# flare-rpc/flare-cpp

Hardware: AMD Instinct MI355X
Metric: GiB/s device-resident Snappy decode+encode, batched RPC bodies, 1/2/4/8 GPU (higher is better)
Workload: dtype u8; 1 GPU; C3 decompress: 65,536 x 64 KiB Zipf-text bodies (~2.0x), device-resident; op=decompress, messages_rank0=65536, global_batch=65536, raw_bytes_all_ranks=4294967296, compressed_bytes_all_ranks=2134156024, parallelism=shard1 (weak: messages by index; no data-path collective), world_size_seen_by_collectives=1

## Files before the change

### flare-cpp_amd/csrc/decode_v4_exec5.h

```cpp
#pragma once

#include "decode_v4_exec_common.h"
#include "decode_v4_plan.h"
#include "snappy_pieces.h"
#include "wave_util.h"

namespace fsg {

namespace {
constexpr u32 kGroupBytes = 1024;

__device__ __forceinline__ u32 exec_tag_entry(u32 c) {
  const u32 type = c & 3, l0 = (c >> 2) + 1;
  u32 nb, len, lit = 0, ll = 0, hi = 0;
  if (type == 0) {
    lit = 1;
    nb = l0 > 60 ? l0 - 60 : 0;
    ll = nb ? 1 : 0;
    len = nb ? 0 : l0;
  } else if (type == 1) {
    nb = 1;
    len = 4 + ((c >> 2) & 7);
    hi = (c >> 5) << 8;
  } else {
    nb = type == 2 ? 2 : 4;
    len = l0;
  }
  return ((32 - 8 * nb) & 31) | (ll << 5) | (lit << 6) | (len << 8) | (nb << 16) | (hi << 20);
}
}

__device__ __forceinline__ void exec5_message(
    u32 m, const u8* __restrict__ in, const u64* __restrict__ in_off,
    const u32* __restrict__ in_len, u8* out, const u64* __restrict__ out_off,
    const u32* __restrict__ out_len, i32* __restrict__ status, const u32* __restrict__ bm_base,
    const u32* __restrict__ bitmap, u32* ring, const u32* tagtab, u8* sb, const u32x4* sel_tab,
    const u32x4* mtab, u32 lane, i32 st, u32 ip0, u32 op0, u32 op1, bool prio, u32 keep_hist) {
  const u32 bmb = bm_base[m];
  const u32 n_in = in_len[m];
  const u32 expected = out_len[m];
  const u8* ib = in + in_off[m];
  u8* ob = out + out_off[m];
  if (st != kOk) return;
  const u32 ibal = (u32)(reinterpret_cast<uintptr_t>(ib) & 15);
  const u32 obal = (u32)(reinterpret_cast<uintptr_t>(ob) & 15);
  const __amdgpu_buffer_rsrc_t irsrc = msg_rsrc(ib - ibal, ibal + n_in);
  const __amdgpu_buffer_rsrc_t orsrc =
      __builtin_amdgcn_make_buffer_rsrc(ob - obal, (short)0, (int)(expected + obal), 0x00020000);

  if ((bmb & kSingleLiteral) && op1 == expected && op0 == 0) {
    const u32 S = bmb & ~kSingleLiteral;
    for (u32 k0 = 0; k0 < expected; k0 += 4096) {
      Raw16 x[4];
#pragma unroll
      for (u32 r = 0; r < 4; ++r) x[r] = raw_load16(irsrc, S + k0 + 1024 * r + lane * 16 + ibal);
#pragma unroll
      for (u32 r = 0; r < 4; ++r) {
        const u32 k = k0 + 1024 * r + lane * 16;
        if (k < expected) store_exact(ob + k, shifted16(x[r]), expected - k < 16 ? expected - k : 16u);
      }
    }
    return;
  }
  const u32* bm = bitmap + bmb;
  const u32 nwords = (n_in + 31) >> 5;
#ifdef FSG_STAMPS
  u64 st_[8] = {0, 0, 0, 0, 0, 0, 0, 0};
  u64 t_last_ = __builtin_amdgcn_s_memtime();
#endif

  u32 head = 0, tail = 0, scan = ip0 >> 5, op = op0;
  int sbase = (int)((op0 + obal) & ~15u) - (int)obal;
  u32 flushed = op0;
  auto zero_from = [&](u32 from) {
    const u32 i = from + 16 * lane;
    if (i < kWindow + 32) *reinterpret_cast<u32x4*>(sb + i) = u32x4{0, 0, 0, 0};
  };
  zero_from(0);
  u32 zero_end = 1024;
  wave_lds_fence();
  auto fill_word = [&](u32 sc) -> u32 {
    const u32 wi = sc + (lane >> 2);
    return (lane < 4 * kFillWords && wi < nwords) ? bm[wi] : 0u;
  };
  u32 bmw = fill_word(scan);
  u32 pf_head = 0xffffffffu, pf_cnt = 0;
  u32 pf_pos = 0;
  u32x4 pd = u32x4{0, 0, 0, 0};
  u32 pd4 = 0;
  auto prefetch = [&](u32 p) {
    const u32 a = (p + ibal) & ~3u;
    pd = __builtin_amdgcn_raw_buffer_load_b128(irsrc, a, 0, 0);
    pd4 = __builtin_amdgcn_raw_buffer_load_b32(irsrc, a + 16, 0, 0);
  };

  auto flush_to = [&](u32 fe) {
    if (fe <= flushed) return;
    const int b0 = (int)(((flushed + obal) & ~15u)) - (int)obal;
    for (int blk = b0 + 16 * (int)lane; blk < (int)fe; blk += 1024) {
      const u32 lo = blk < (int)flushed ? flushed : (u32)blk;
      const u32 hi = blk + 16 < (int)fe ? (u32)(blk + 16) : fe;
      if (hi - lo == 16) {
        const u32x4 v = *reinterpret_cast<const u32x4*>(sb + (blk - sbase));
        __builtin_memcpy(ob + blk, &v, 16);
      } else {
        store_exact(ob + lo, lds_read16(sb + ((int)lo - sbase)), hi - lo);
      }
    }
    flushed = fe;
  };

  for (;;) {
    if (tail - head < 2 * kMaxPieces && scan < nwords) {
      if (prio) __builtin_amdgcn_s_setprio(1);
      u32 bits = (bmw >> (8 * (lane & 3))) & 0xffu;
      const u32 bitbase = (scan + (lane >> 2)) * 32 + 8 * (lane & 3);
      if (bitbase < ip0) bits &= bitbase + 8 <= ip0 ? 0u : (0xffu << (ip0 - bitbase)) & 0xffu;
      const u32 cnt = __builtin_popcount(bits);
      const u32 incl = dpp_incl_scan(cnt);
      u32 slot = tail + incl - cnt;
      while (bits) {
        ring[slot & (kTagRing - 1)] = bitbase + __builtin_ctz(bits);
        ++slot;
        bits &= bits - 1;
      }
      tail += readlane(incl, 63);
      scan += kFillWords;
      bmw = fill_word(scan);
      wave_lds_fence();
      STAMP(0);
      continue;
    }
    const u32 avail = tail - head;
    if (avail == 0 || op >= op1) break;
    const u32 take0 = avail < 64 ? avail : 64u;
    const bool valid = lane < take0;
    const u32 pos = ring[(head + lane) & (kTagRing - 1)];
    if (pf_head != head || pf_cnt < take0) prefetch(pos);
    if (prio) __builtin_amdgcn_s_setprio(1);

    const u32 s = (pos + ibal) & 3u;
    const u32 c = __builtin_amdgcn_alignbyte(pd[1], pd[0], s) & 0xffu;
    const u32 e = tagtab[c];
    const bool q = s == 3;
    const u32 w0 = q ? pd[1] : pd[0], w1 = q ? pd[2] : pd[1], w2 = q ? pd[3] : pd[2];
    const u32 w3 = q ? pd4 : pd[3];
    const u32 b = (s + 1) & 3u;
    const u32x4 xr = u32x4{__builtin_amdgcn_alignbyte(w1, w0, b), __builtin_amdgcn_alignbyte(w2, w1, b),
                           __builtin_amdgcn_alignbyte(w3, w2, b), __builtin_amdgcn_alignbyte(pd4, w3, b)};
    const u32 val = xr[0] & (0xffffffffu >> (e & 31u));
    const bool is_lit = e & 64u;
    const u32 len = (e & 32u) ? val + 1u : (e >> 8) & 0x7fu;
    const u32 off = val + (e >> 20);
    const u32 nb = (e >> 16) & 7u;
    const u32 lsrc = pos + 1 + nb;

    const u64 bigm = __ballot(valid && is_lit && len > 64);
    STAMP(1);
    if (bigm & 1ull) {
      const u32 L = readlane(len, 0), S = readlane(lsrc, 0);
      if ((u64)op + L > op1) {
        if (lane == 0) status[m] = kCorrupt;
        return;
      }
      flush_to(op);
      for (u32 k0 = 0; k0 < L; k0 += 4096) {
        Raw16 x[4];
#pragma unroll
        for (u32 r = 0; r < 4; ++r) x[r] = raw_load16(irsrc, S + k0 + 1024 * r + lane * 16 + ibal);
#pragma unroll
        for (u32 r = 0; r < 4; ++r) {
          const u32 k = k0 + 1024 * r + lane * 16;
          if (k < L) store_exact(ob + op + k, shifted16(x[r]), L - k < 16 ? L - k : 16u);
        }
      }
      op += L;
      flushed = op;
      sbase = (int)((op + obal) & ~15u) - (int)obal - 16;
      zero_from(0);
      zero_end = 1024;
      wave_lds_fence();
      if (lane < 2) {
        const u32 lo = (u32)sbase + 16 * lane;
        if (lo < op) {
          const u32 cnt = op - lo < 16 ? op - lo : 16u;
          store_exact(sb + 16 * lane, rsrc_load16(irsrc, S + L - (op - lo) + ibal), cnt);
        }
      }
      wave_lds_fence();
      head += 1;
      pf_head = 0xffffffffu;
      if (head == tail) {
        const u32 nw = (S + L) >> 5;
        if (nw > scan) {
          scan = nw;
          bmw = fill_word(scan);
        }
      }
      STAMP(7);
      continue;
    }
    const u32 take = bigm ? (u32)__builtin_ctzll(bigm) : take0;
    const bool v = lane < take;

    const u32 lv = v ? len : 0u;
    const u32 incl = dpp_incl_scan(lv);
    const u32 t_op = op + incl - lv;
    const bool fits = v && incl <= kGroupBytes && t_op < op1;
    const u32 k_tags = (u32)__builtin_popcountll(__ballot(fits));
    const u32 tot_len = readlane(incl, k_tags - 1);
    if (__any(fits && (len > op1 - t_op || (!is_lit && (off == 0 || off > t_op - op0))))) {
      if (lane == 0) status[m] = kCorrupt;
      return;
    }

    if (op + tot_len - sbase > kWindow) {
      const int nsb = (int)(((op - keep_hist + obal) & ~15u)) - (int)obal;
      if ((int)flushed < nsb + 16) flush_to((u32)((int)((op + obal) & ~15u) - (int)obal));
      wait_all_memory();
      const u32 shift = (u32)(nsb - sbase), keep = (u32)((int)op - nsb);
      for (u32 k = 0; k < keep; k += 1024) {
        const u32 i = k + 16 * lane;
        u32x4 x = u32x4{0, 0, 0, 0};
        if (i < keep) x = *reinterpret_cast<const u32x4*>(sb + shift + i);
        wave_lds_fence();
        if (i < keep) *reinterpret_cast<u32x4*>(sb + i) = x;
        wave_lds_fence();
      }
      sbase = nsb;
      zero_end = (keep + 15) & ~15u;
    }
    auto prefetch_next_and_zero = [&]() {
      {
        const u32 nh = head + k_tags;
        const u32 na = tail - nh;
        const u32 ncnt = na < 64 ? na : 64u;
        pf_pos = ring[(nh + lane) & (kTagRing - 1)];
        prefetch(pf_pos);
        pf_head = nh;
        pf_cnt = ncnt;
      }
      while (op + tot_len + 20 - sbase > zero_end) {
        zero_from(zero_end);
        zero_end += 1024;
      }
      wave_lds_fence();
    };

    STAMP(2);
    const u32 src = is_lit ? lsrc : t_op - off;
    const u32 nch = (len + 15) >> 4;
    const bool pat = !is_lit && off < 16 && off < len;
    const u32 below = (u32)(sbase - (int)src);
    const u32 kfar = (int)below > 0 ? ((below - 1) >> 4) + 1 : 0u;
    const u32 kready = src + len <= op ? nch : (src < op ? (op - src) >> 4 : 0u);
    const u32 klead = kfar > kready ? kfar : kready;
    const u32 kc = pat ? 0u : (klead < nch ? klead : nch);
    const u32 kf = fits ? (is_lit ? nch : kc) : 0u;
    const bool reg0 = is_lit && nb == 0;
    const u32 sh = is_lit ? (src + ibal) & 3u : 0u;
    auto gload = [&](u32 k, u32x4& d, u32& d4) {
      if (is_lit) {
        const u32 a = (src + 16 * k + ibal) & ~3u;
        d = __builtin_amdgcn_raw_buffer_load_b128(irsrc, a, 0, 0);
        d4 = __builtin_amdgcn_raw_buffer_load_b32(irsrc, a + 16, 0, 0);
      } else if (k >= kfar) {
        d = lds_read16(sb + ((int)(src + 16 * k) - sbase));
      } else {
        d = far_load(orsrc, src + 16 * k + obal);
      }
    };
    u32x4 a0 = xr, a1 = u32x4{0, 0, 0, 0};
    u32 a0e = 0, a1e = 0;
    if (kf > 0 && !reg0) gload(0, a0, a0e);
    const u64 m1 = __ballot(kf > 1);
    if (m1 && kf > 1) gload(1, a1, a1e);
    prefetch_next_and_zero();
    if (prio) __builtin_amdgcn_s_setprio(0);
    STAMP(3);
    {
      const int fe = (int)((op + obal) & ~15u) - (int)obal;
      if (fe >= (int)flushed + 1024) flush_to((u32)fe);
    }
    STAMP(4);
    const u32 wa = (u32)((int)t_op - sbase);
    if (kf > 0) or_store(sb, wa, shift16(a0, a0e, reg0 ? 0u : sh), len < 16 ? len : 16u, mtab);
    if (m1) {
      if (kf > 1) or_store(sb, wa + 16, shift16(a1, a1e, sh), len - 16 < 16 ? len - 16 : 16u, mtab);
      if (__ballot(kf > 2)) {
        if (kf > 2) gload(2, a0, a0e);
        if (kf > 3) gload(3, a1, a1e);
        if (kf > 2) or_store(sb, wa + 32, shift16(a0, a0e, sh), len - 32 < 16 ? len - 32 : 16u, mtab);
        if (kf > 3) or_store(sb, wa + 48, shift16(a1, a1e, sh), len - 48, mtab);
      }
    }
    wave_lds_fence();

    STAMP(5);
    u32 rem = (fits && kf < nch) ? len - 16 * kf : 0u;
    u32 cw = (u32)((int)t_op - sbase) + 16 * kf;
    u32 sw = (u32)((int)src - sbase) + 16 * kf;
    const u32 stp = pat ? pat_step(off) : 16u;
    u32 n = rem < stp ? rem : stp;
    bool pf = pat;
    u32 ne = rem ? (pf ? cw : sw + n) : 0xffffffffu;
    u64 pend = __ballot(rem > 0);
    if (!__ballot(pat && rem > 0)) {
      while (pend) {
        const u32 W = readlane(cw, (u32)__builtin_ctzll(pend));
        if (ne <= W) {
          const u32x4 x = lds_read16(sb + sw);
          const u32x4 o = lds_read16(sb + cw);
          const u32x4 y = merge16(x, o, mtab[n]);
          __builtin_memcpy(sb + cw, &y, 16);
          rem -= n;
          cw += n;
          sw += n;
          n = rem < 16u ? rem : 16u;
          ne = rem ? sw + n : 0xffffffffu;
        }
        wave_lds_fence();
        pend = __ballot(rem > 0);
      }
    }
    while (pend) {
      const u32 W = readlane(cw, (u32)__builtin_ctzll(pend));
      if (ne <= W) {
        u32x4 x = lds_read16(sb + sw);
        if (pf) x = expand_pattern(x, off, sel_tab);
        const u32x4 o = lds_read16(sb + cw);
        const u32x4 y = merge16(x, o, mtab[n]);
        __builtin_memcpy(sb + cw, &y, 16);
        rem -= n;
        cw += n;
        sw = pat ? cw - stp : sw + n;
        pf = false;
        n = rem < stp ? rem : stp;
        ne = rem ? sw + n : 0xffffffffu;
      }
      wave_lds_fence();
      pend = __ballot(rem > 0);
    }
    op += tot_len;
    head += k_tags;
    STAMP(6);
  }
  if (op != op1) {
    if (lane == 0) status[m] = kCorrupt;
    return;
  }
  flush_to(op1);
#ifdef FSG_STAMPS
  if (lane == 0)
    for (int k = 0; k < 8; ++k) atomicAdd(&g_stamps[k], (unsigned long long)st_[k]);
#endif
}

}
```

### flare-cpp_amd/csrc/decode_v4_plan.h

```cpp
#pragma once

#include <stddef.h>
#include <stdint.h>

namespace fsg {

typedef uint8_t u8;
typedef uint32_t u32;
typedef uint64_t u64;
typedef int64_t i64;

#ifndef FSG_IDX_WAVES
#define FSG_IDX_WAVES 1
#endif
constexpr u32 kIdxWaves = FSG_IDX_WAVES;
static_assert(kIdxWaves == 1 || kIdxWaves == 2 || kIdxWaves == 4, "tag table init");
#ifndef FSG_IDX_WAVES_SERIAL
#define FSG_IDX_WAVES_SERIAL 4
#endif
constexpr u32 kIdxWavesSerial = FSG_IDX_WAVES_SERIAL;
static_assert(kIdxWavesSerial == 1 || kIdxWavesSerial == 2 || kIdxWavesSerial == 4, "tag table init");
constexpr u32 kWalkClasses = 16;
constexpr u32 kPlanThreads = 1024;

constexpr u32 kBigIndexMin = 8 * 1024;
constexpr u32 kBigIndexMax = 48 * 1024;
#ifndef FSG_HUGE_KB
#define FSG_HUGE_KB 256
#endif
constexpr u32 kHugeIndexBytes = FSG_HUGE_KB * 1024;
constexpr u32 kChunkBytes = 32 * 1024;
struct ChunkRec {
  u32 m, k, exit, bad, len, base, flags, nchunks;
};

constexpr u32 kWavesPerBlock = 4;
constexpr u32 kSingleLiteral = 0x80000000u;
#ifndef FSG_WINDOW
#define FSG_WINDOW 3072
#define FSG_KEEP 1024
#endif
constexpr u32 kWindow = FSG_WINDOW;
constexpr u32 kKeep = FSG_KEEP;
constexpr u32 kMaxKeep = (kWindow - 16 * 64 - 48) & ~15u;
static_assert(kKeep <= kMaxKeep, "kept history leaves room for one group");
constexpr u32 kPackCtrWide = 3, kPackCtrGuard = 4;

constexpr u32 kWsBmCounter = 0;
constexpr u32 kWsSet1BigNext = 16;
constexpr u32 kWsSet1SegCount = 32;
constexpr u32 kWsSet1WholeCount = 48;
constexpr u32 kWsBigCount = 64;
constexpr u32 kWsHugeCount = kWsBigCount + 32;
constexpr u32 kWsSet0BigNext = 128;
constexpr u32 kWsSet0SegCount = 160;
constexpr u32 kWsSet0ExecNext = 192;
constexpr u32 kWsSet0WholeCount = 224;
constexpr u32 kWsSet1ExecNext = 240;
constexpr u32 kWsChunkCount = 80;
constexpr u32 kWsChunkSpecNext = 84;
constexpr u32 kWsChunkFixNext = 88;
constexpr u32 kWsChunkCheckNext = 92;
constexpr u32 kWsChunkFinalNext = 100;
constexpr u32 kWsPackNext = 104;
constexpr u32 kWsFallbackCount = 108;
constexpr u32 kWsFallbackBitmap = 112;
constexpr u32 kWsFallbackWide = kWsPackNext + 4 * kPackCtrWide;
constexpr u32 kWsFallbackGuard = kWsPackNext + 4 * kPackCtrGuard;
static_assert(kWsFallbackBitmap == kWsFallbackCount + 4, "fallback_kernel counts at fb_count[0..1]");
constexpr u32 kWsCounterBytes = 256;
constexpr u32 kWsOffsets[] = {kWsBmCounter, kWsSet1BigNext, kWsSet1SegCount, kWsSet1WholeCount, kWsBigCount,
                              kWsHugeCount, kWsSet0BigNext, kWsSet0SegCount, kWsSet0ExecNext, kWsSet0WholeCount,
                              kWsSet1ExecNext, kWsChunkCount, kWsChunkSpecNext, kWsChunkFixNext,
                              kWsChunkCheckNext, kWsChunkFinalNext, kWsPackNext, kWsFallbackCount,
                              kWsFallbackBitmap, kWsFallbackWide, kWsFallbackGuard};
constexpr bool ws_offsets_ok() {
  for (u32 i = 0; i < sizeof(kWsOffsets) / sizeof(kWsOffsets[0]); ++i) {
    if (kWsOffsets[i] % 4 || kWsOffsets[i] + 4 > kWsCounterBytes) return false;
    for (u32 j = 0; j < i; ++j)
      if (kWsOffsets[i] < kWsOffsets[j] + 4 && kWsOffsets[j] < kWsOffsets[i] + 4) return false;
  }
  return true;
}
static_assert(ws_offsets_ok(), "workspace counters overlap or leave the header");
constexpr u64 kListBases = 11;
constexpr u64 kChunkRegionDiv = 64;
inline size_t decode_v4_workspace_bytes(u32 n_msgs, u64 total_in_bytes) {
  const u64 base_bytes = (4ull * n_msgs + 255) & ~255ull;
  const u64 words = total_in_bytes / 32 + 4ull * n_msgs + 64;
  const u64 base = 256 + kListBases * base_bytes + 4 * words;
  return (size_t)(base + base / (kChunkRegionDiv - 1) + 512);
}

inline u64 decode_v4_bitmap_capacity_words(u32 n_msgs, size_t ws_bytes) {
  const u64 base_bytes = (4ull * n_msgs + 255) & ~255ull;
  const u64 chunk_bytes = (ws_bytes / kChunkRegionDiv) & ~255ull;
  const u64 chunk_off = (ws_bytes - chunk_bytes) & ~255ull;
  u64 cap_words = (chunk_off - 256 - kListBases * base_bytes) / 4;
  if (cap_words >= kSingleLiteral) cap_words = kSingleLiteral - 1;
  return cap_words;
}

constexpr size_t idx_lean_lds_bytes() { return 4 * (kIdxWaves * (8 * 4 + 5 + 8) * 64 + 256); }

struct DecodeOpts {
  i64 decode_fork = -1;
  i64 split_walk = 3;
  i64 split_class = 4;
  i64 exec_keep = -1;
  i64 chunked_huge = 1;
  i64 small_persist = 3584;
  i64 small_batch = 64;
  i64 split_huge = 1;
  i64 walk_order = 1;
  i64 lean_walk = 1;
  i64 exec_big_blocks = 512;
  i64 exec_prio = 1;
  i64 exec_big_blocks_fork = 1024;
  i64 exec_pack = 32;
};

struct LaunchDim {
  u32 grid, block, lds;
};
enum WalkKind : int {
  kWalkPlanned,
  kWalkLean,
  kWalkSerial,
  kWalkStandard,
};

struct DecodePlan {
  u64 base_bytes;
  u64 bm_base_off, big_list_off, seg_list_off, whole_list_off, walk_rank_off, walk_perm_off, walk_hist_off,
      seg_list2_off, whole_list2_off;
  u64 bitmap_off;
  u64 cap_words;
  u64 chunk_off, chunk_bytes;
  u64 first_rec_off, mstat_off, recs_off;
  u64 max_huge, max_recs;
  bool chunked;
  u64 est_total_in;
  u32 big_threshold;
  bool split_huge, walk_order, fork;
  u32 split_mode, split_class, prio, keep_hist, pack_batch;
  WalkKind walk_kind;
  LaunchDim walk;
  LaunchDim planned_walk;
  u32 plan_grid;
  u32 scatter_grid;
  u32 index_big_grid;
  u32 small_blocks;
  u32 big_blocks;
  u32 fork_big_blocks;
  u32 small_grid;
  u32 small_stride;
  u32 chunk_list_grid, chunk_rec_grid, chunk_msg_grid;
  u32 fallback_grid;
};

inline DecodePlan decode_v4_plan(u32 n_msgs, size_t ws_bytes, bool two_stream, const DecodeOpts& o) {
  DecodePlan p{};
  p.split_huge = o.split_huge != 0;
  p.walk_order = o.walk_order != 0;
  const bool lean_walk = o.lean_walk != 0;
  const u64 base_bytes = (4ull * n_msgs + 255) & ~255ull;
  p.base_bytes = base_bytes;
  p.bm_base_off = 256;
  p.big_list_off = 256 + base_bytes;
  p.seg_list_off = 256 + 2 * base_bytes;
  p.whole_list_off = 256 + 4 * base_bytes;
  p.walk_rank_off = 256 + 5 * base_bytes;
  p.walk_perm_off = 256 + 6 * base_bytes;
  p.walk_hist_off = 256 + 7 * base_bytes;
  p.seg_list2_off = 256 + 8 * base_bytes;
  p.whole_list2_off = 256 + 10 * base_bytes;
  p.bitmap_off = 256 + kListBases * base_bytes;
  const u64 chunk_bytes = (ws_bytes / kChunkRegionDiv) & ~255ull;
  const u64 chunk_off = (ws_bytes - chunk_bytes) & ~255ull;
  p.chunk_bytes = chunk_bytes;
  p.chunk_off = chunk_off;
  const u64 cap_words = decode_v4_bitmap_capacity_words(n_msgs, ws_bytes);
  p.cap_words = cap_words;
  const u64 est_total_in = cap_words > 4ull * n_msgs + 64 ? (cap_words - 4ull * n_msgs - 64) * 32 : 0;
  p.est_total_in = est_total_in;
  u64 thr = 4 * est_total_in / n_msgs;
  thr = thr < kBigIndexMin ? kBigIndexMin : (thr > kBigIndexMax ? kBigIndexMax : thr);
  if ((i64)n_msgs <= o.small_batch) thr = 0;
  p.big_threshold = (u32)thr;
  const u32 idx_blocks = (n_msgs + 64 * kIdxWaves - 1) / (64 * kIdxWaves);
  p.split_mode = (u32)o.split_walk;
  p.split_class = (u32)o.split_class % kWalkClasses;
  p.planned_walk = LaunchDim{idx_blocks, 64 * kIdxWaves, 0u};
  if (two_stream && lean_walk) {
    p.walk_kind = kWalkLean;
    p.walk = LaunchDim{idx_blocks, 64 * kIdxWaves, (u32)idx_lean_lds_bytes()};
  } else if (est_total_in < 16384ull * n_msgs) {
    p.walk_kind = kWalkSerial;
    p.walk = LaunchDim{(n_msgs + 64 * kIdxWavesSerial - 1) / (64 * kIdxWavesSerial), 64 * kIdxWavesSerial, 0u};
  } else {
    p.walk_kind = kWalkStandard;
    p.walk = LaunchDim{idx_blocks, 64 * kIdxWaves, 0u};
  }
  const u32 small_blocks = (n_msgs + kWavesPerBlock - 1) / kWavesPerBlock;
  p.small_blocks = small_blocks;
  const i64 big_opt = o.exec_big_blocks;
  const u32 big_blocks_opt = big_opt >= 1 && big_opt <= (1 << 20) ? (u32)big_opt : 512u;
  p.prio = o.exec_prio != 0 ? 1u : 0u;
  p.keep_hist = kKeep;
  {
    const i64 v = o.exec_keep;
    if (v >= 512 && v <= (i64)kMaxKeep && v % 16 == 0) p.keep_hist = (u32)v;
  }
  const i64 fork_opt = o.decode_fork;
  p.fork = !two_stream && (fork_opt >= 0 ? fork_opt != 0 : n_msgs > 131072u);
  p.big_blocks = small_blocks < big_blocks_opt ? small_blocks : big_blocks_opt;
  {
    const u32 q = (n_msgs + 3) / 4;
    p.index_big_grid = q < 1024u ? q : 1024u;
  }
  const i64 bbf_opt = o.exec_big_blocks_fork;
  const u32 big_blocks_fork_opt = bbf_opt >= 1 && bbf_opt <= (1 << 20) ? (u32)bbf_opt : 1024u;
  p.fork_big_blocks = small_blocks < big_blocks_fork_opt ? small_blocks : big_blocks_fork_opt;
  const bool chunked_opt = o.chunked_huge != 0;
  const u64 max_huge_need = est_total_in / kHugeIndexBytes + 1;
  const u64 max_huge = 8 * max_huge_need < chunk_bytes ? max_huge_need : chunk_bytes / 320;
  const u64 max_recs = max_huge ? (chunk_bytes - 8 * max_huge) / sizeof(ChunkRec) : 0;
  p.max_huge = max_huge;
  p.max_recs = max_recs;
  p.first_rec_off = chunk_off;
  p.mstat_off = chunk_off + 4 * max_huge;
  p.recs_off = chunk_off + 8 * max_huge;
  p.chunked = chunked_opt && max_huge >= est_total_in / kHugeIndexBytes + 1 &&
              max_recs >= est_total_in / kChunkBytes + est_total_in / kHugeIndexBytes + 2;
  {
    const u32 lb = (u32)((max_huge + 255) / 256);
    p.chunk_list_grid = lb ? lb : 1u;
    p.chunk_rec_grid = (u32)(max_recs / 4 + 1 < 1024 ? max_recs / 4 + 1 : 1024);
    p.chunk_msg_grid = (u32)(max_huge / 4 + 1 < 256 ? max_huge / 4 + 1 : 256);
  }
  const i64 sp_opt = o.small_persist;
  const u32 small_persist = sp_opt >= 0 && sp_opt <= (1 << 20) ? (u32)sp_opt : 3584u;
  p.small_grid = small_persist && small_persist < small_blocks ? small_persist : small_blocks;
  p.small_stride = p.small_grid < small_blocks ? p.small_grid : 0u;
  const i64 pack_opt = o.exec_pack;
  p.pack_batch = pack_opt >= 1 && pack_opt <= 64 ? (u32)pack_opt : 0u;
  p.plan_grid = (n_msgs + kPlanThreads - 1) / kPlanThreads;
  p.scatter_grid = (n_msgs + 255) / 256;
  p.fallback_grid = (n_msgs + 63) / 64;
  return p;
}

}
```

### flare-cpp_amd/csrc/snappy_decode_v4.hip

```cpp
#include "options.h"
#include "snappy_lane_decode.h"
#include "snappy_pieces.h"
#include "wave_util.h"

#include <mutex>

#include "decode_v4_plan.h"
#include "launch.h"
#include "launch_util.h"

#include "decode_v4_index.h"
#include "decode_v4_index_big.h"
#include "decode_v4_chunked.h"
#include "decode_v4_exec4.h"
#include "decode_v4_exec5.h"
#include "decode_v4_packed.h"

namespace fsg {

static_assert(kWave == 64, "idx_lean_lds_bytes (decode_v4_plan.h) counts 64 lanes per wave");

#ifndef FSG_EXEC_WAVES
#define FSG_EXEC_WAVES 7
#endif
template <int V>
__global__ __launch_bounds__(kWavesPerBlock * 64) __attribute__((amdgpu_waves_per_eu(FSG_EXEC_WAVES, FSG_EXEC_WAVES))) void exec_kernel(
    const u8* __restrict__ in, const u64* __restrict__ in_off,
    const u32* __restrict__ in_len, u32 n_msgs, u8* out,
    const u64* __restrict__ out_off, const u32* __restrict__ out_len,
    i32* __restrict__ status, const u32* __restrict__ bm_base,
    u32* __restrict__ bitmap, const u32* __restrict__ seg_list,
    const u32* __restrict__ seg_count, const u32* __restrict__ whole_list,
    const u32* __restrict__ whole_count, u32* __restrict__ exec_next, u32 big_blocks,
    u32 big_threshold, u32 prio, u32 keep_hist, u32 small_stride, const u32* __restrict__ walk_perm = nullptr,
    const u32* __restrict__ walk_hist = nullptr, u32 walk_part = 0, u32 split_class = 0) {
  __shared__ __attribute__((aligned(16))) u8 wl_s[kWavesPerBlock][4 * kTagRing + kWindow + 32];
  __shared__ __attribute__((aligned(16))) u8 pmap_s[kWavesPerBlock][V == 5 ? 1 : kMaxPieces];
  __shared__ u32x4 sel_tab[16];
  __shared__ u32 tagtab[V == 5 ? 256 : 1];
  __shared__ u32x4 mask_tab[17];
  static_assert(kWavesPerBlock * 64 == 256, "one tag table entry per thread");

  if (threadIdx.x < 64) init_pattern_table(sel_tab, threadIdx.x);
  if constexpr (V == 5) tagtab[threadIdx.x] = exec_tag_entry(threadIdx.x);
  init_mask_table(mask_tab, threadIdx.x);
  __syncthreads();
  auto run = [&](u32 m, u32* ring, u8* pmap, u8* sb, u32 lane, i32 st, u32 ip0, u32 op0, u32 op1) {
    if constexpr (V == 5)
      exec5_message(m, in, in_off, in_len, out, out_off, out_len, status, bm_base, bitmap, ring, tagtab,
                    sb, sel_tab, mask_tab, lane, st, ip0, op0, op1, prio != 0, keep_hist);
    else
      exec_message(m, in, in_off, in_len, out, out_off, out_len, status, bm_base, bitmap, ring, pmap,
                   sb, sel_tab, mask_tab, lane, st, ip0, op0, op1, prio != 0, keep_hist);
  };

  const u32 wv = (u32)__builtin_amdgcn_readfirstlane((int)(threadIdx.x >> 6));
  const u32 lane = threadIdx.x & 63;
  u32* ring = reinterpret_cast<u32*>(wl_s[wv]);
  u8* pmap = pmap_s[wv];
  u8* sb = wl_s[wv] + 4 * kTagRing;

  if (blockIdx.x >= big_blocks) {
    const u32 m0 = (blockIdx.x - big_blocks) * kWavesPerBlock + wv;
    const u32 step = small_stride ? small_stride * kWavesPerBlock : 0xffffffffu;
    if (walk_perm) {
      const u32 n_walk = walk_hist[2 * kWalkClasses];
      const u32 tcls = split_class >> 8;
      const u32 split = walk_hist[kWalkClasses + (split_class & 0xffu)];
      const u32 t_hi = tcls ? walk_hist[kWalkClasses + tcls] : n_walk;
      const u32 lo = walk_part == 2 ? split : 0u, hi = walk_part == 1 ? split : t_hi;
      for (u32 i = m0; i < hi - lo; i = i + step < i ? 0xffffffffu : i + step) {
        const u32 m = walk_perm[lo + i];
        run(m, ring, pmap, sb, lane, status[m], 0u, 0u, out_len[m]);
      }
      return;
    }
    for (u32 m = m0; m < n_msgs; m = m + step < m ? 0xffffffffu : m + step)
      if (in_len[m] <= big_threshold) run(m, ring, pmap, sb, lane, status[m], 0u, 0u, out_len[m]);
    return;
  }
  const u32 n_whole = *whole_count;
  const u32 n_seg_raw = *seg_count;
  const u32 n_seg = n_seg_raw < n_msgs ? n_seg_raw : n_msgs;
  const u32 total = n_whole + n_seg;
  if (total == 0) return;
  const u64* segs = reinterpret_cast<const u64*>(seg_list);
  for (;;) {
    const u32 got = atomicAdd(exec_next, lane == 0 ? 1u : 0u);
    const u32 idx = (u32)__builtin_amdgcn_readfirstlane((int)got);
    if (idx >= total) break;
    if (idx < n_whole) {
      const u32 m = whole_list[idx];
      run(m, ring, pmap, sb, lane, status[m], 0u, 0u, out_len[m]);
      continue;
    }
    const u64 e = segs[idx - n_whole];
    const u32 m = (u32)e;
    if (m == 0xffffffffu) continue;
    const u32 k = (u32)(e >> 32) & 0x7fffffffu;
    const u32 expected = out_len[m];
    const u32 op0 = k << 16;
    const u32 op1 = (e >> 63) ? expected : op0 + 65536u;
    u32 ip0 = 0;
    if (k) __builtin_memcpy(&ip0, out + out_off[m] + op0, 4);
    run(m, ring, pmap, sb, lane, status[m], ip0, op0, op1);
  }
}

#ifndef FSG_PACK_WAVES
#define FSG_PACK_WAVES 6
#endif
__global__ __launch_bounds__(kWavesPerBlock * 64) __attribute__((amdgpu_waves_per_eu(FSG_PACK_WAVES, FSG_PACK_WAVES))) void exec_packed_kernel(
    const u8* __restrict__ in, const u64* __restrict__ in_off, const u32* __restrict__ in_len, u8* out,
    const u64* __restrict__ out_off, const u32* __restrict__ out_len, i32* __restrict__ status,
    const u32* __restrict__ bm_base, const u32* __restrict__ bitmap, const u32* __restrict__ walk_perm,
    const u32* __restrict__ walk_hist, u32 split_class, u32* __restrict__ batch_next, u32 batch, u32 keep_hist) {
  __shared__ __attribute__((aligned(16))) u8 wl_s[kWavesPerBlock][4 * kTagRing + kWindow + 32];
  __shared__ u32x4 sel_tab[16];
  __shared__ u32 tagtab[256];
  __shared__ u32x4 mask_tab[17];
  static_assert(kWavesPerBlock * 64 == 256, "one tag table entry per thread");
  if (threadIdx.x < 64) init_pattern_table(sel_tab, threadIdx.x);
  tagtab[threadIdx.x] = exec_tag_entry(threadIdx.x);
  init_mask_table(mask_tab, threadIdx.x);
  __syncthreads();
  const u32 wv = (u32)__builtin_amdgcn_readfirstlane((int)(threadIdx.x >> 6));
  const u32 lane = threadIdx.x & 63;
  u32* ring = reinterpret_cast<u32*>(wl_s[wv]);
  u8* sb = wl_s[wv] + 4 * kTagRing;
  const u32 n_walk = walk_hist[2 * kWalkClasses];
  const u32 tcls = split_class >> 8;
  const u32 lo = walk_hist[kWalkClasses + (split_class & 0xffu)];
  const u32 hi = tcls ? walk_hist[kWalkClasses + tcls] : n_walk;
  const u32 n = hi > lo ? hi - lo : 0u;
  for (;;) {
    const u32 got = atomicAdd(batch_next, lane == 0 ? 1u : 0u);
    const u32 bi = (u32)__builtin_amdgcn_readfirstlane((int)got);
    if ((u64)bi * batch >= n) break;
    const u32 first = bi * batch;
    const u32 cnt = n - first < batch ? n - first : batch;
    exec5_packed(in, in_off, in_len, out, out_off, out_len, status, bm_base, bitmap, walk_perm, lo + first, cnt,
                 ring, tagtab, sb, sel_tab, mask_tab, lane, keep_hist, batch_next);
  }
}

#ifdef FSG_STAMPS
extern "C" int fsg_debug_stamps(unsigned long long* out, int reset) {
  hipError_t e = hipMemcpyFromSymbol(out, HIP_SYMBOL(g_stamps), sizeof(g_stamps));
  if (reset) {
    unsigned long long z[24] = {};
    (void)hipMemcpyToSymbol(HIP_SYMBOL(g_stamps), z, sizeof(z));
  }
  return e == hipSuccess ? 0 : -1;
}
#endif

__global__ __launch_bounds__(64) void fallback_kernel(
    const u8* __restrict__ in, const u64* __restrict__ in_off, const u32* __restrict__ in_len,
    u32 n_msgs, u8* out, const u64* __restrict__ out_off, const u32* __restrict__ out_len,
    i32* __restrict__ status, u32 flags, const u32* __restrict__ bm_base, u64 bm_capacity_words,
    u32* __restrict__ fb_count) {
  const u32 m = blockIdx.x * 64 + threadIdx.x;
  const bool mine = m < n_msgs && status[m] == kNeedFallback;
  const u64 fb = __ballot(mine);
  if (!fb) return;
  const u32 n_in = mine ? in_len[m] : 0u;
  const u32 bmb = mine ? bm_base[m] : 0u;
  const u32 words = (((n_in + 31) >> 5) + 3) & ~3u;
  const u64 fb_bm = __ballot(mine && !(bmb & kSingleLiteral) && (u64)bmb + words > bm_capacity_words);
  if (threadIdx.x == 0) {
    atomicAdd(fb_count, (u32)__builtin_popcountll(fb));
    if (fb_bm) atomicAdd(fb_count + 1, (u32)__builtin_popcountll(fb_bm));
  }
  if (!mine) return;
  const u8* ib = in + in_off[m];
  u32 ulen = 0;
  const int h = parse_varint_header(ib, n_in, flags & 2u, &ulen);
  status[m] = decode_one(ib + h, ib + n_in, out + out_off[m], out_len[m], true);
}

void decode_v4_header_counts(const void* header, DecodeHeaderCounts* c) {
  u32 ctr[kWsCounterBytes / 4];
  __builtin_memcpy(ctr, header, sizeof(ctr));
  auto at = [&ctr](u32 off) { return ctr[off / 4]; };
  c->bitmap_words = at(kWsBmCounter);
  c->large = at(kWsBigCount);
  c->huge = at(kWsHugeCount);
  c->fallback = at(kWsFallbackCount);
  c->fallback_bitmap = at(kWsFallbackBitmap);
  c->fallback_wide = at(kWsFallbackWide);
  c->fallback_guard = at(kWsFallbackGuard);
}

namespace {

struct SideStream {
  hipStream_t stream = nullptr;
  hipStream_t stream2 = nullptr;
  hipEvent_t join2 = nullptr;
  hipStream_t stream3 = nullptr;
  hipEvent_t join3 = nullptr;
  hipEvent_t fork = nullptr, join = nullptr;
  hipEvent_t pass1 = nullptr;
  std::mutex mu;
};
bool create_side_stream(SideStream* s) {
  if (hipStreamCreateWithFlags(&s->stream, hipStreamNonBlocking) != hipSuccess ||
      hipEventCreateWithFlags(&s->fork, hipEventDisableTiming) != hipSuccess ||
      hipEventCreateWithFlags(&s->join, hipEventDisableTiming) != hipSuccess ||
      hipEventCreateWithFlags(&s->pass1, hipEventDisableTiming) != hipSuccess)
    return false;
  if (hipStreamCreateWithFlags(&s->stream2, hipStreamNonBlocking) != hipSuccess ||
      hipEventCreateWithFlags(&s->join2, hipEventDisableTiming) != hipSuccess)
    s->stream2 = nullptr;
  if (hipStreamCreateWithFlags(&s->stream3, hipStreamNonBlocking) != hipSuccess ||
      hipEventCreateWithFlags(&s->join3, hipEventDisableTiming) != hipSuccess)
    s->stream3 = nullptr;
  return true;
}
SideStream* side_stream() { return per_device<SideStream>(create_side_stream); }

struct BigSet {
  u32 *big_next, *seg_count, *whole_count, *exec_next;
  u64* seg_list;
  u32* whole_list;
};

using ExecKernel = decltype(&exec_kernel<5>);
ExecKernel exec_kernel_variant(int v) { return v == 4 ? &exec_kernel<4> : &exec_kernel<5>; }

struct DecodeBufs {
  const u8* in;
  const u64* in_off;
  const u32* in_len;
  u32 n_msgs;
  u8* out;
  const u64* out_off;
  const u32* out_cap;
  u32* out_len;
  i32* status;
  u32 flags;
  ExecKernel ek;
  u8* w;
  u32 *counter, *big_count, *bm_base, *big_list;
  u32 *walk_rank, *walk_perm, *walk_hist;
  u32* bitmap;
  BigSet set0, set1;
  u32 *first_rec, *mstat;
  ChunkRec* recs;
  u32* ctr(u32 off) const { return reinterpret_cast<u32*>(w + off); }
};

void workspace_pointers(const DecodePlan& p, void* ws, DecodeBufs* b) {
  u8* w = static_cast<u8*>(ws);
  auto words = [w](u64 off) { return reinterpret_cast<u32*>(w + off); };
  b->w = w;
  b->counter = words(kWsBmCounter);
  b->big_count = words(kWsBigCount);
  b->bm_base = words(p.bm_base_off);
  b->big_list = words(p.big_list_off);
  b->walk_rank = words(p.walk_rank_off);
  b->walk_perm = words(p.walk_perm_off);
  b->walk_hist = words(p.walk_hist_off);
  b->bitmap = words(p.bitmap_off);
  b->set0 = BigSet{words(kWsSet0BigNext), words(kWsSet0SegCount), words(kWsSet0WholeCount), words(kWsSet0ExecNext),
                   reinterpret_cast<u64*>(w + p.seg_list_off), words(p.whole_list_off)};
  b->set1 = BigSet{words(kWsSet1BigNext), words(kWsSet1SegCount), words(kWsSet1WholeCount), words(kWsSet1ExecNext),
                   reinterpret_cast<u64*>(w + p.seg_list2_off), words(p.whole_list2_off)};
  b->first_rec = words(p.first_rec_off);
  b->mstat = words(p.mstat_off);
  b->recs = reinterpret_cast<ChunkRec*>(w + p.recs_off);
}

hipError_t launch_index(const DecodePlan& p, const DecodeBufs& b, bool planned, hipStream_t st, u32 part = 0) {
  const LaunchDim& d = planned ? p.planned_walk : p.walk;
  if (planned)
    index_kernel<true><<<d.grid, d.block, d.lds, st>>>(
        b.in, b.in_off, b.in_len, b.n_msgs, b.out_cap, b.out_len, b.status, b.flags, b.counter, b.bm_base, b.bitmap,
        p.cap_words, b.big_count, b.big_list, p.big_threshold, p.walk_order ? b.walk_perm : nullptr, b.walk_hist,
        part, p.split_class);
  else if (p.walk_kind == kWalkLean)
    index_kernel<false, true><<<d.grid, d.block, d.lds, st>>>(
        b.in, b.in_off, b.in_len, b.n_msgs, b.out_cap, b.out_len, b.status, b.flags, b.counter, b.bm_base, b.bitmap,
        p.cap_words, b.big_count, b.big_list, p.big_threshold, nullptr, nullptr);
  else if (p.walk_kind == kWalkSerial)
    index_kernel<false, false, kIdxWavesSerial><<<d.grid, d.block, d.lds, st>>>(
        b.in, b.in_off, b.in_len, b.n_msgs, b.out_cap, b.out_len, b.status, b.flags, b.counter, b.bm_base, b.bitmap,
        p.cap_words, b.big_count, b.big_list, p.big_threshold, nullptr, nullptr);
  else
    index_kernel<false><<<d.grid, d.block, d.lds, st>>>(
        b.in, b.in_off, b.in_len, b.n_msgs, b.out_cap, b.out_len, b.status, b.flags, b.counter, b.bm_base, b.bitmap,
        p.cap_words, b.big_count, b.big_list, p.big_threshold, nullptr, nullptr);
  return hipGetLastError();
}

hipError_t launch_index_big(const DecodePlan& p, const DecodeBufs& b, hipStream_t st, const BigSet& s, u32 mode) {
  index_big_kernel<<<p.index_big_grid, 256, 0, st>>>(
      b.in, b.in_off, b.in_len, b.out_len, b.flags, b.status, b.bm_base, b.bitmap, b.big_count, b.big_list,
      s.big_next, b.n_msgs, b.out, b.out_off, s.seg_list, s.seg_count, s.whole_list, s.whole_count, mode);
  return hipGetLastError();
}

hipError_t launch_big_exec(const DecodePlan& p, const DecodeBufs& b, hipStream_t st, const BigSet& s) {
  b.ek<<<p.fork_big_blocks, kWavesPerBlock * 64, 0, st>>>(
      b.in, b.in_off, b.in_len, b.n_msgs, b.out, b.out_off, b.out_len, b.status, b.bm_base, b.bitmap,
      reinterpret_cast<const u32*>(s.seg_list), s.seg_count, s.whole_list, s.whole_count, s.exec_next,
      p.fork_big_blocks, p.big_threshold, 0u, p.keep_hist, 0u, nullptr, nullptr, 0u, 0u);
  return hipGetLastError();
}

hipError_t launch_big(const DecodePlan& p, const DecodeBufs& b, hipStream_t st, const BigSet& s, u32 mode) {
  const hipError_t e = launch_index_big(p, b, st, s, mode);
  if (e != hipSuccess) return e;
  return launch_big_exec(p, b, st, s);
}

hipError_t launch_big_chunked(const DecodePlan& p, const DecodeBufs& b, hipStream_t st, const BigSet& s) {
  u32* const cctr = b.ctr(kWsChunkCount);
  chunk_list_kernel<<<p.chunk_list_grid, 256, 0, st>>>(b.in, b.in_off, b.in_len, b.big_count, b.big_list, b.n_msgs,
                                                       b.flags, cctr, b.recs, b.first_rec, (u32)p.max_recs);
  chunk_spec_kernel<<<p.chunk_rec_grid, 256, 0, st>>>(b.in, b.in_off, b.in_len, b.flags, b.bm_base, b.bitmap, cctr,
                                                      b.recs, b.ctr(kWsChunkSpecNext), (u32)p.max_recs);
  chunk_fixup_kernel<<<p.chunk_msg_grid, 256, 0, st>>>(b.in, b.in_off, b.in_len, b.out_len, b.bm_base, b.bitmap,
                                                       b.big_count, b.recs, b.first_rec, b.mstat,
                                                       b.ctr(kWsChunkFixNext));
  chunk_check_kernel<<<p.chunk_rec_grid, 256, 0, st>>>(b.in, b.in_off, b.in_len, b.out_len, b.bm_base, b.bitmap, cctr,
                                                       b.recs, b.out, b.out_off, b.ctr(kWsChunkCheckNext),
                                                       (u32)p.max_recs);
  chunk_final_kernel<<<p.chunk_msg_grid, 256, 0, st>>>(b.in, b.in_off, b.in_len, b.flags, b.bm_base, b.bitmap, b.out,
                                                       b.out_off, b.big_list, b.out_len, b.status, b.big_count,
                                                       b.recs, b.first_rec, b.mstat, b.n_msgs, s.seg_list,
                                                       s.seg_count, s.whole_list, s.whole_count,
                                                       b.ctr(kWsChunkFinalNext));
  const hipError_t e = hipGetLastError();
  if (e != hipSuccess) return e;
  return launch_big_exec(p, b, st, s);
}

hipError_t launch_small(const DecodePlan& p, const DecodeBufs& b, hipStream_t st, u32 part) {
  b.ek<<<p.small_grid, kWavesPerBlock * 64, 0, st>>>(
      b.in, b.in_off, b.in_len, b.n_msgs, b.out, b.out_off, b.out_len, b.status, b.bm_base, b.bitmap,
      reinterpret_cast<const u32*>(b.set0.seg_list), b.set0.seg_count, b.set0.whole_list, b.set0.whole_count,
      b.set0.exec_next, 0u, p.big_threshold, 0u, p.keep_hist, p.small_stride, part ? b.walk_perm : nullptr,
      part ? b.walk_hist : nullptr, part, p.split_class);
  return hipGetLastError();
}

hipError_t launch_packed(const DecodePlan& p, const DecodeBufs& b, hipStream_t st) {
  exec_packed_kernel<<<p.small_grid, kWavesPerBlock * 64, 0, st>>>(
      b.in, b.in_off, b.in_len, b.out, b.out_off, b.out_len, b.status, b.bm_base, b.bitmap, b.walk_perm, b.walk_hist,
      p.split_class, b.ctr(kWsPackNext), p.pack_batch, p.keep_hist);
  return hipGetLastError();
}

hipError_t launch_forked(const DecodePlan& p, const DecodeBufs& b, SideStream* side, hipStream_t stream) {
  hipError_t e;
  index_plan_kernel<<<p.plan_grid, kPlanThreads, 0, stream>>>(
      b.in, b.in_off, b.in_len, b.n_msgs, b.out_cap, b.out_len, b.status, b.flags, b.counter, b.bm_base, b.bitmap,
      p.cap_words, b.big_count, b.big_list, p.big_threshold, p.walk_order ? b.walk_rank : nullptr, b.walk_hist);
  if ((e = hipGetLastError()) != hipSuccess) return e;
  if (p.walk_order) {
    walk_offsets_kernel<<<1, 64, 0, stream>>>(b.walk_hist);
    walk_scatter_kernel<<<p.scatter_grid, 256, 0, stream>>>(b.in_len, b.n_msgs, b.status, b.walk_rank, b.walk_hist,
                                                            b.walk_perm);
    if ((e = hipGetLastError()) != hipSuccess) return e;
  }
  std::lock_guard<std::mutex> lk(side->mu);
  if ((e = hipEventRecord(side->fork, stream)) != hipSuccess) return e;
  if ((e = hipStreamWaitEvent(side->stream, side->fork, 0)) != hipSuccess) return e;
  const bool split = p.split_huge && side->stream2;
  if (split) {
    if ((e = hipStreamWaitEvent(side->stream2, side->fork, 0)) != hipSuccess) return e;
    if ((e = p.chunked ? launch_big_chunked(p, b, side->stream2, b.set1)
                       : launch_big(p, b, side->stream2, b.set1, 1u)) != hipSuccess)
      return e;
    if ((e = hipEventRecord(side->join2, side->stream2)) != hipSuccess) return e;
  }
  if ((e = launch_big(p, b, side->stream, b.set0, split ? 2u : 0u)) != hipSuccess) return e;
  if ((e = hipEventRecord(side->join, side->stream)) != hipSuccess) return e;
  const bool three = p.split_mode == 1 && p.walk_order && side->stream3;
  if (three) {
    if ((e = hipStreamWaitEvent(side->stream3, side->fork, 0)) != hipSuccess) return e;
    if ((e = launch_index(p, b, true, side->stream3, 1u)) != hipSuccess) return e;
    if ((e = launch_small(p, b, side->stream3, 1u)) != hipSuccess) return e;
    if ((e = hipEventRecord(side->join3, side->stream3)) != hipSuccess) return e;
    if ((e = launch_index(p, b, true, stream, 2u)) != hipSuccess) return e;
    if ((e = launch_small(p, b, stream, 2u)) != hipSuccess) return e;
    if ((e = hipStreamWaitEvent(stream, side->join3, 0)) != hipSuccess) return e;
  } else {
    if ((e = launch_index(p, b, true, stream)) != hipSuccess) return e;
    if (p.walk_order && p.split_mode == 2) {
      if ((e = launch_small(p, b, stream, 3u)) != hipSuccess) return e;
    } else if (p.walk_order && p.split_mode == 3) {
      if ((e = p.pack_batch ? launch_packed(p, b, stream) : launch_small(p, b, stream, 2u)) != hipSuccess) return e;
      if ((e = launch_small(p, b, stream, 1u)) != hipSuccess) return e;
    } else {
      if ((e = launch_small(p, b, stream, 0u)) != hipSuccess) return e;
    }
  }
  if ((e = hipStreamWaitEvent(stream, side->join, 0)) != hipSuccess) return e;
  if (split && (e = hipStreamWaitEvent(stream, side->join2, 0)) != hipSuccess) return e;
  return hipSuccess;
}

DecodeOpts read_decode_opts() {
  DecodeOpts o;
  o.decode_fork = opt(kOptDecodeFork);
  o.split_walk = opt(kOptSplitWalk);
  o.split_class = opt(kOptSplitClass);
  o.exec_keep = opt(kOptExecKeep);
  o.chunked_huge = opt(kOptChunkedHuge);
  o.small_persist = opt(kOptSmallPersist);
  o.small_batch = opt(kOptSmallBatch);
  o.split_huge = opt(kOptSplitHuge);
  o.walk_order = opt(kOptWalkOrder);
  o.lean_walk = opt(kOptLeanWalk);
  o.exec_big_blocks = opt(kOptExecBigBlocks);
  o.exec_prio = opt(kOptExecPrio);
  o.exec_big_blocks_fork = opt(kOptExecBigBlocksFork);
  o.exec_pack = opt(kOptExecPack);
  return o;
}

}

hipError_t launch_decode_v4(const u8* in, const u64* in_off, const u32* in_len,
                            u32 n_msgs, u8* out, const u64* out_off,
                            const u32* out_cap, u32* out_len, i32* status,
                            u32 flags, void* ws, size_t ws_bytes, hipStream_t stream,
                            int exec_variant, hipStream_t pass1_stream) {
  if (n_msgs == 0) return hipSuccess;
  SideStream* two = nullptr;
  if (pass1_stream && pass1_stream != stream) {
    two = side_stream();
    if (!two) {
      const hipError_t e0 = order_after(stream, pass1_stream);
      if (e0 != hipSuccess) return e0;
    }
  }
  if (ws_bytes < decode_v4_workspace_bytes(n_msgs, 0)) return hipErrorInvalidValue;

  const DecodePlan p = decode_v4_plan(n_msgs, ws_bytes, two != nullptr, read_decode_opts());
  DecodeBufs b{in, in_off, in_len, n_msgs, out, out_off, out_cap, out_len, status, flags,
               exec_kernel_variant(exec_variant)};
  workspace_pointers(p, ws, &b);

  hipStream_t const s1 = two ? pass1_stream : stream;
  hipError_t e = hipMemsetAsync(b.w, 0, p.bitmap_off, s1);
  if (e != hipSuccess) return e;

  SideStream* side = p.fork ? side_stream() : nullptr;
  if (side) {
    if ((e = launch_forked(p, b, side, stream)) != hipSuccess) return e;
  } else {
    if ((e = launch_index(p, b, false, s1)) != hipSuccess) return e;
    if ((e = launch_index_big(p, b, s1, b.set0, 0u)) != hipSuccess) return e;
    if (two) {
      std::lock_guard<std::mutex> lk(two->mu);
      if ((e = hipEventRecord(two->pass1, s1)) != hipSuccess) return e;
      if ((e = hipStreamWaitEvent(stream, two->pass1, 0)) != hipSuccess) return e;
    }
    b.ek<<<p.big_blocks + p.small_blocks, kWavesPerBlock * 64, 0, stream>>>(
        in, in_off, in_len, n_msgs, out, out_off, out_len, status, b.bm_base, b.bitmap,
        reinterpret_cast<const u32*>(b.set0.seg_list), b.set0.seg_count, b.set0.whole_list, b.set0.whole_count,
        b.set0.exec_next, p.big_blocks, p.big_threshold, p.prio, p.keep_hist, 0u, nullptr, nullptr, 0u, 0u);
    if ((e = hipGetLastError()) != hipSuccess) return e;
  }
  fallback_kernel<<<p.fallback_grid, 64, 0, stream>>>(in, in_off, in_len, n_msgs, out, out_off, out_len, status,
                                                      flags, b.bm_base, p.cap_words, b.ctr(kWsFallbackCount));
  return hipGetLastError();
}

}
```

Measured before the change: 703.4 GiB/s (uncompressed bytes).

## Use 16-bit tag ring for whole small messages to enlarge LDS output window

For small messages decoded whole, the exec5 path is templated to store tag positions in a 16-bit ring. The LDS bytes this frees are handed to a larger staging window (kWindow + 1024), with a larger default kept history packed into the upper half of keep_hist. The aim is fewer window slides, with their flush, wait and LDS copy, per 64 KiB body. Segmented big messages keep the 32-bit ring. The cost is a second template instance, which adds code size and may change register allocation.

```diff
diff --git a/flare-cpp_amd/csrc/decode_v4_exec5.h b/flare-cpp_amd/csrc/decode_v4_exec5.h
--- a/flare-cpp_amd/csrc/decode_v4_exec5.h
+++ b/flare-cpp_amd/csrc/decode_v4_exec5.h
@@ -9,6 +9,7 @@
 
 namespace {
 constexpr u32 kGroupBytes = 1024;
+static_assert(kExecRing == kTagRing, "decode_v4_plan.h sizes the folded instance's window from the ring");
 
 __device__ __forceinline__ u32 exec_tag_entry(u32 c) {
   const u32 type = c & 3, l0 = (c >> 2) + 1;
@@ -30,15 +31,21 @@
 }
 }
 
+template <bool kWhole, typename RingT, u32 kWin>
 __device__ __forceinline__ void exec5_message(
     u32 m, const u8* __restrict__ in, const u64* __restrict__ in_off,
     const u32* __restrict__ in_len, u8* out, const u64* __restrict__ out_off,
     const u32* __restrict__ out_len, i32* __restrict__ status, const u32* __restrict__ bm_base,
-    const u32* __restrict__ bitmap, u32* ring, const u32* tagtab, u8* sb, const u32x4* sel_tab,
-    const u32x4* mtab, u32 lane, i32 st, u32 ip0, u32 op0, u32 op1, bool prio, u32 keep_hist) {
+    const u32* __restrict__ bitmap, RingT* ring, const u32* tagtab, u8* sb, const u32x4* sel_tab,
+    const u32x4* mtab, u32 lane, i32 st, u32 ip0_, u32 op0_, u32 op1_, bool prio, u32 keep_hist) {
+  static_assert(sizeof(RingT) == 4 || (kWhole && sizeof(RingT) == 2 && kBigIndexMax < 65536),
+                "16-bit ring entries: tag positions of a body of at most big_threshold bytes");
+  static_assert(sizeof(RingT) * kTagRing + kWin == 4 * kTagRing + kWindow && kWin % 16 == 0,
+                "ring + window fill the wave's LDS");
   const u32 bmb = bm_base[m];
   const u32 n_in = in_len[m];
   const u32 expected = out_len[m];
+  const u32 ip0 = kWhole ? 0u : ip0_, op0 = kWhole ? 0u : op0_, op1 = kWhole ? expected : op1_;
   const u8* ib = in + in_off[m];
   u8* ob = out + out_off[m];
   if (st != kOk) return;
@@ -74,7 +81,7 @@
   u32 flushed = op0;
   auto zero_from = [&](u32 from) {
     const u32 i = from + 16 * lane;
-    if (i < kWindow + 32) *reinterpret_cast<u32x4*>(sb + i) = u32x4{0, 0, 0, 0};
+    if (i < kWin + 32) *reinterpret_cast<u32x4*>(sb + i) = u32x4{0, 0, 0, 0};
   };
   zero_from(0);
   u32 zero_end = 1024;
@@ -120,7 +127,7 @@
       const u32 incl = dpp_incl_scan(cnt);
       u32 slot = tail + incl - cnt;
       while (bits) {
-        ring[slot & (kTagRing - 1)] = bitbase + __builtin_ctz(bits);
+        ring[slot & (kTagRing - 1)] = (RingT)(bitbase + __builtin_ctz(bits));
         ++slot;
         bits &= bits - 1;
       }
@@ -214,7 +221,7 @@
       return;
     }
 
-    if (op + tot_len - sbase > kWindow) {
+    if (op + tot_len - sbase > kWin) {
       const int nsb = (int)(((op - keep_hist + obal) & ~15u)) - (int)obal;
       if ((int)flushed < nsb + 16) flush_to((u32)((int)((op + obal) & ~15u) - (int)obal));
       wait_all_memory();
diff --git a/flare-cpp_amd/csrc/decode_v4_plan.h b/flare-cpp_amd/csrc/decode_v4_plan.h
--- a/flare-cpp_amd/csrc/decode_v4_plan.h
+++ b/flare-cpp_amd/csrc/decode_v4_plan.h
@@ -44,6 +44,19 @@
 constexpr u32 kKeep = FSG_KEEP;
 constexpr u32 kMaxKeep = (kWindow - 16 * 64 - 48) & ~15u;
 static_assert(kKeep <= kMaxKeep, "kept history leaves room for one group");
+constexpr u32 kExecRing = 512;
+static_assert(kBigIndexMax < 65536, "the folded instance's ring entries are 16 bits");
+constexpr u32 kWindowWhole = kWindow + 2 * kExecRing;
+#ifndef FSG_KEEP_WHOLE
+#define FSG_KEEP_WHOLE 2048
+#endif
+constexpr u32 kKeepWhole = FSG_KEEP_WHOLE;
+constexpr u32 kMaxKeepWhole = (kWindowWhole - 16 * 64 - 48) & ~15u;
+static_assert(kKeepWhole <= kMaxKeepWhole && kKeepWhole % 16 == 0, "kept history leaves room for one group");
+constexpr u32 exec_wave_lds_bytes(bool whole) {
+  return (whole ? 2 * kExecRing + kWindowWhole : 4 * kExecRing + kWindow) + 32;
+}
+static_assert(exec_wave_lds_bytes(true) == exec_wave_lds_bytes(false), "one LDS carve-up per wave");
 constexpr u32 kPackCtrWide = 3, kPackCtrGuard = 4;
 
 constexpr u32 kWsBmCounter = 0;
@@ -143,7 +156,7 @@
   u64 est_total_in;
   u32 big_threshold;
   bool split_huge, walk_order, fork;
-  u32 split_mode, split_class, prio, keep_hist, pack_batch;
+  u32 split_mode, split_class, prio, keep_hist, keep_hist_whole, pack_batch;
   WalkKind walk_kind;
   LaunchDim walk;
   LaunchDim planned_walk;
@@ -208,9 +221,11 @@
   const u32 big_blocks_opt = big_opt >= 1 && big_opt <= (1 << 20) ? (u32)big_opt : 512u;
   p.prio = o.exec_prio != 0 ? 1u : 0u;
   p.keep_hist = kKeep;
+  p.keep_hist_whole = kKeepWhole;
   {
     const i64 v = o.exec_keep;
     if (v >= 512 && v <= (i64)kMaxKeep && v % 16 == 0) p.keep_hist = (u32)v;
+    if (v >= 512 && v <= (i64)kMaxKeepWhole && v % 16 == 0) p.keep_hist_whole = (u32)v;
   }
   const i64 fork_opt = o.decode_fork;
   p.fork = !two_stream && (fork_opt >= 0 ? fork_opt != 0 : n_msgs > 131072u);
diff --git a/flare-cpp_amd/csrc/snappy_decode_v4.hip b/flare-cpp_amd/csrc/snappy_decode_v4.hip
--- a/flare-cpp_amd/csrc/snappy_decode_v4.hip
+++ b/flare-cpp_amd/csrc/snappy_decode_v4.hip
@@ -4,6 +4,7 @@
 #include "wave_util.h"
 
 #include <mutex>
+#include <type_traits>
 
 #include "decode_v4_plan.h"
 #include "launch.h"
@@ -45,38 +46,42 @@
   if constexpr (V == 5) tagtab[threadIdx.x] = exec_tag_entry(threadIdx.x);
   init_mask_table(mask_tab, threadIdx.x);
   __syncthreads();
-  auto run = [&](u32 m, u32* ring, u8* pmap, u8* sb, u32 lane, i32 st, u32 ip0, u32 op0, u32 op1) {
-    if constexpr (V == 5)
-      exec5_message(m, in, in_off, in_len, out, out_off, out_len, status, bm_base, bitmap, ring, tagtab,
-                    sb, sel_tab, mask_tab, lane, st, ip0, op0, op1, prio != 0, keep_hist);
-    else
-      exec_message(m, in, in_off, in_len, out, out_off, out_len, status, bm_base, bitmap, ring, pmap,
-                   sb, sel_tab, mask_tab, lane, st, ip0, op0, op1, prio != 0, keep_hist);
-  };
-
   const u32 wv = (u32)__builtin_amdgcn_readfirstlane((int)(threadIdx.x >> 6));
   const u32 lane = threadIdx.x & 63;
-  u32* ring = reinterpret_cast<u32*>(wl_s[wv]);
+  u8* wl = wl_s[wv];
   u8* pmap = pmap_s[wv];
-  u8* sb = wl_s[wv] + 4 * kTagRing;
+  auto run = [&](auto whole, u32 m, i32 st, u32 ip0, u32 op0, u32 op1) {
+    constexpr bool kWhole = decltype(whole)::value;
+    if constexpr (V == 5 && kWhole)
+      exec5_message<true, u16, kWindowWhole>(m, in, in_off, in_len, out, out_off, out_len, status, bm_base, bitmap,
+                                             reinterpret_cast<u16*>(wl), tagtab, wl + 2 * kTagRing, sel_tab,
+                                             mask_tab, lane, st, 0u, 0u, 0u, prio != 0, keep_hist >> 16);
+    else if constexpr (V == 5)
+      exec5_message<false, u32, kWindow>(m, in, in_off, in_len, out, out_off, out_len, status, bm_base, bitmap,
+                                         reinterpret_cast<u32*>(wl), tagtab, wl + 4 * kTagRing, sel_tab, mask_tab,
+                                         lane, st, ip0, op0, op1, prio != 0, keep_hist & 0xffffu);
+    else
+      exec_message(m, in, in_off, in_len, out, out_off, out_len, status, bm_base, bitmap,
+                   reinterpret_cast<u32*>(wl), pmap, wl + 4 * kTagRing, sel_tab, mask_tab, lane, st, ip0, op0, op1,
+                   prio != 0, keep_hist & 0xffffu);
+  };
 
   if (blockIdx.x >= big_blocks) {
     const u32 m0 = (blockIdx.x - big_blocks) * kWavesPerBlock + wv;
     const u32 step = small_stride ? small_stride * kWavesPerBlock : 0xffffffffu;
+    u32 lo = 0, n = n_msgs;
     if (walk_perm) {
       const u32 n_walk = walk_hist[2 * kWalkClasses];
       const u32 tcls = split_class >> 8;
       const u32 split = walk_hist[kWalkClasses + (split_class & 0xffu)];
       const u32 t_hi = tcls ? walk_hist[kWalkClasses + tcls] : n_walk;
-      const u32 lo = walk_part == 2 ? split : 0u, hi = walk_part == 1 ? split : t_hi;
-      for (u32 i = m0; i < hi - lo; i = i + step < i ? 0xffffffffu : i + step) {
-        const u32 m = walk_perm[lo + i];
-        run(m, ring, pmap, sb, lane, status[m], 0u, 0u, out_len[m]);
-      }
-      return;
-    }
-    for (u32 m = m0; m < n_msgs; m = m + step < m ? 0xffffffffu : m + step)
-      if (in_len[m] <= big_threshold) run(m, ring, pmap, sb, lane, status[m], 0u, 0u, out_len[m]);
+      lo = walk_part == 2 ? split : 0u;
+      n = (walk_part == 1 ? split : t_hi) - lo;
+    }
+    for (u32 i = m0; i < n; i = i + step < i ? 0xffffffffu : i + step) {
+      const u32 m = walk_perm ? walk_perm[lo + i] : i;
+      if (in_len[m] <= big_threshold) run(std::true_type{}, m, status[m], 0u, 0u, out_len[m]);
+    }
     return;
   }
   const u32 n_whole = *whole_count;
@@ -89,21 +94,20 @@
     const u32 got = atomicAdd(exec_next, lane == 0 ? 1u : 0u);
     const u32 idx = (u32)__builtin_amdgcn_readfirstlane((int)got);
     if (idx >= total) break;
+    u32 m, ip0 = 0, op0 = 0, op1;
     if (idx < n_whole) {
-      const u32 m = whole_list[idx];
-      run(m, ring, pmap, sb, lane, status[m], 0u, 0u, out_len[m]);
-      continue;
-    }
-    const u64 e = segs[idx - n_whole];
-    const u32 m = (u32)e;
-    if (m == 0xffffffffu) continue;
-    const u32 k = (u32)(e >> 32) & 0x7fffffffu;
-    const u32 expected = out_len[m];
-    const u32 op0 = k << 16;
-    const u32 op1 = (e >> 63) ? expected : op0 + 65536u;
-    u32 ip0 = 0;
-    if (k) __builtin_memcpy(&ip0, out + out_off[m] + op0, 4);
-    run(m, ring, pmap, sb, lane, status[m], ip0, op0, op1);
+      m = whole_list[idx];
+      op1 = out_len[m];
+    } else {
+      const u64 e = segs[idx - n_whole];
+      m = (u32)e;
+      if (m == 0xffffffffu) continue;
+      const u32 k = (u32)(e >> 32) & 0x7fffffffu;
+      op0 = k << 16;
+      op1 = (e >> 63) ? out_len[m] : op0 + 65536u;
+      if (k) __builtin_memcpy(&ip0, out + out_off[m] + op0, 4);
+    }
+    run(std::false_type{}, m, status[m], ip0, op0, op1);
   }
 }
 
@@ -228,6 +232,7 @@
 
 using ExecKernel = decltype(&exec_kernel<5>);
 ExecKernel exec_kernel_variant(int v) { return v == 4 ? &exec_kernel<4> : &exec_kernel<5>; }
+u32 exec_keep_arg(const DecodePlan& p) { return p.keep_hist | (p.keep_hist_whole << 16); }
 
 struct DecodeBufs {
   const u8* in;
@@ -305,7 +310,7 @@
   b.ek<<<p.fork_big_blocks, kWavesPerBlock * 64, 0, st>>>(
       b.in, b.in_off, b.in_len, b.n_msgs, b.out, b.out_off, b.out_len, b.status, b.bm_base, b.bitmap,
       reinterpret_cast<const u32*>(s.seg_list), s.seg_count, s.whole_list, s.whole_count, s.exec_next,
-      p.fork_big_blocks, p.big_threshold, 0u, p.keep_hist, 0u, nullptr, nullptr, 0u, 0u);
+      p.fork_big_blocks, p.big_threshold, 0u, exec_keep_arg(p), 0u, nullptr, nullptr, 0u, 0u);
   return hipGetLastError();
 }
 
@@ -341,7 +346,7 @@
   b.ek<<<p.small_grid, kWavesPerBlock * 64, 0, st>>>(
       b.in, b.in_off, b.in_len, b.n_msgs, b.out, b.out_off, b.out_len, b.status, b.bm_base, b.bitmap,
       reinterpret_cast<const u32*>(b.set0.seg_list), b.set0.seg_count, b.set0.whole_list, b.set0.whole_count,
-      b.set0.exec_next, 0u, p.big_threshold, 0u, p.keep_hist, p.small_stride, part ? b.walk_perm : nullptr,
+      b.set0.exec_next, 0u, p.big_threshold, 0u, exec_keep_arg(p), p.small_stride, part ? b.walk_perm : nullptr,
       part ? b.walk_hist : nullptr, part, p.split_class);
   return hipGetLastError();
 }
@@ -463,7 +468,7 @@
     b.ek<<<p.big_blocks + p.small_blocks, kWavesPerBlock * 64, 0, stream>>>(
         in, in_off, in_len, n_msgs, out, out_off, out_len, status, b.bm_base, b.bitmap,
         reinterpret_cast<const u32*>(b.set0.seg_list), b.set0.seg_count, b.set0.whole_list, b.set0.whole_count,
-        b.set0.exec_next, p.big_blocks, p.big_threshold, p.prio, p.keep_hist, 0u, nullptr, nullptr, 0u, 0u);
+        b.set0.exec_next, p.big_blocks, p.big_threshold, p.prio, exec_keep_arg(p), 0u, nullptr, nullptr, 0u, 0u);
     if ((e = hipGetLastError()) != hipSuccess) return e;
   }
   fallback_kernel<<<p.fallback_grid, 64, 0, stream>>>(in, in_off, in_len, n_msgs, out, out_off, out_len, status,
```

Result: faster. 727.0 GiB/s (uncompressed bytes), median of 6 (+3.3%).
